# zyc-123/InstanceDiff

Measured on AMD Instinct MI355X. Metric: denoising steps/sec (256x256 bs16), higher is better.
Workload: dtype f32; 1 GPU; 256x256 1-ch synthetic, 1000-step reverse chain, batch 16 per GPU, 2 UNet fwd + reverse update per step; global_batch=16, parallelism=replicas x1 (no collective)

## Files before the change

instancediff_amd/csrc/conv1x1_x3.hip:

```cpp
#include "conv_args.h"
#include "wino_common.h"

using idiff_detail::ConvArgs;

namespace {

typedef unsigned uintx4 __attribute__((ext_vector_type(4)));
typedef __bf16 bf16x8 __attribute__((ext_vector_type(8)));

constexpr int BM = 64, CKB = 32, NT = 256;
constexpr int B_ISTR = 1088;
constexpr int B_KGSTR = 4 * B_ISTR;
constexpr int B_PLSTR = 4 * B_KGSTR;
constexpr int B_BYTES = 3 * B_PLSTR;
constexpr int A_PLSTR = 4 * 64 * 16;
constexpr int A_BYTES = 3 * A_PLSTR;
constexpr int OLD = 256 + 4;
static_assert(32 * OLD * 4 <= B_BYTES, "epilogue tile must fit in the B planes");

__host__ __device__ constexpr unsigned hi16(unsigned u) { return u & 0xffff0000u; }

__device__ __forceinline__ unsigned pack_hi(unsigned odd, unsigned even) { return __builtin_amdgcn_perm(odd, even, 0x07060302u); }

__device__ __forceinline__ void split3(const float (&x)[8], uintx4& p1, uintx4& p2, uintx4& p3) {
    unsigned u1[8], u2[8], u3[8];
#pragma unroll
    for (int c = 0; c < 8; ++c) {
        u1[c] = __builtin_bit_cast(unsigned, x[c]);
        const float r1 = x[c] - __builtin_bit_cast(float, hi16(u1[c]));
        u2[c] = __builtin_bit_cast(unsigned, r1);
        const float r2 = r1 - __builtin_bit_cast(float, hi16(u2[c]));
        u3[c] = __builtin_bit_cast(unsigned, r2);
    }
    p1 = uintx4{pack_hi(u1[1], u1[0]), pack_hi(u1[3], u1[2]), pack_hi(u1[5], u1[4]), pack_hi(u1[7], u1[6])};
    p2 = uintx4{pack_hi(u2[1], u2[0]), pack_hi(u2[3], u2[2]), pack_hi(u2[5], u2[4]), pack_hi(u2[7], u2[6])};
    p3 = uintx4{pack_hi(u3[1], u3[0]), pack_hi(u3[3], u3[2]), pack_hi(u3[5], u3[4]), pack_hi(u3[7], u3[6])};
}

using idiff_wino::scalar_ptr;

__device__ __forceinline__ floatx4 mma(const uintx4& a, const uintx4& b, const floatx4& c) {
    return __builtin_amdgcn_mfma_f32_16x16x32_bf16(__builtin_bit_cast(bf16x8, a), __builtin_bit_cast(bf16x8, b), c, 0, 0, 0);
}

template <bool UNSH>
__global__ __launch_bounds__(NT) __attribute__((amdgpu_waves_per_eu(2, 2))) void conv1x1_x3_kernel(const ConvArgs a, const unsigned short* __restrict__ wx3) {
    extern __shared__ __attribute__((aligned(16))) unsigned char smem_raw[];
    unsigned char* const Bs = smem_raw;
    unsigned char* const As = smem_raw + B_BYTES;
    float* const econst = reinterpret_cast<float*>(smem_raw + B_BYTES + A_BYTES);

    const int tid = threadIdx.x;
    const int lane = tid & 63;
    const int wave = __builtin_amdgcn_readfirstlane(tid >> 6);
    const int n16 = lane & 15, kgl = lane >> 4;

    const unsigned logical = xcd_remap(blockIdx.x, a.total_wg);
    const int cob = logical % a.ncob;
    const int tile = (logical / a.ncob) % a.ntiles;
    const int b = logical / (a.ncob * a.ntiles);
    const int co0 = cob * BM;
    const long long HW = (long long)a.Hout * a.Wout;
    const long long pix0 = (long long)tile * 256;

    {
        const int which = tid >> 6, co = co0 + (tid & 63);
        float v = 0.f;
        if (which == 0 && a.bias) v = a.bias[co];
        if (which == 1 && a.vec) v = a.vec[(long long)b * a.Cout + co];
        if (which == 2 && a.aux) v = a.aux_a[(long long)b * a.Cout + co];
        if (which == 3 && a.aux) v = a.aux_b[(long long)b * a.Cout + co];
        econst[tid] = v;
    }

    const int q = lane, kg = wave;
    const int nchunks = (a.Cin + CKB - 1) / CKB;
    floatx4 xrA[8], xrB[8];
    uintx4 ar[3];
    constexpr int RSRC_FLAGS = 0x00020000;
    const float* const s0 = a.src0 + (long long)b * a.bs0 + (UNSH ? 0 : pix0);
    const float* const s1 = a.src1 ? a.src1 + (long long)b * a.bs1 + pix0 : s0;
    const long long HWin = (long long)a.Hin * a.Win;
    const int chstride_b = (int)((UNSH ? HWin : HW) * 4);
    int xoff = q * 16;
    if (UNSH) {
        const int p = (int)pix0 + 4 * q;
        const int oy = p / a.Wout, ox = p - oy * a.Wout;
        xoff = (2 * oy * a.Win + 2 * ox) * 4;
    }
    auto load_x = [&](floatx4 (&xr)[8], int cc) {
        const int ch0 = cc * CKB + kg * 8;
        const bool valid = ch0 < a.Cin;
        if (UNSH) {
            const float* const p = s0 + (long long)(valid ? (ch0 >> 2) : 0) * HWin;
            const __amdgpu_buffer_rsrc_t rs = __builtin_amdgcn_make_buffer_rsrc(scalar_ptr(p), 0, __builtin_amdgcn_readfirstlane(valid ? 0x7fffffff : 0), RSRC_FLAGS);
#pragma unroll
            for (int c = 0; c < 8; ++c)
                xr[c] = __builtin_bit_cast(floatx4, __builtin_amdgcn_raw_buffer_load_b128(rs, xoff, (c >> 2) * chstride_b + ((c >> 1) & 1) * a.Win * 4 + (c & 1) * 16, 0));
        } else {
            const bool second = ch0 >= a.C0v;
            const float* const p = (second ? s1 : s0) + (long long)(valid ? (second ? ch0 - a.C0v : ch0) : 0) * HW;
            const __amdgpu_buffer_rsrc_t rs = __builtin_amdgcn_make_buffer_rsrc(scalar_ptr(p), 0, __builtin_amdgcn_readfirstlane(valid ? 0x7fffffff : 0), RSRC_FLAGS);
#pragma unroll
            for (int c = 0; c < 8; ++c) xr[c] = __builtin_bit_cast(floatx4, __builtin_amdgcn_raw_buffer_load_b128(rs, xoff, c * chstride_b, 0));
        }
    };
    auto load_w = [&](int cc) {
        const bool valid = cc < nchunks;
        const unsigned short* const wsrc = wx3 + ((long long)(valid ? cc : 0) * a.ncob + cob) * (A_BYTES / 2);
        const __amdgpu_buffer_rsrc_t rs = __builtin_amdgcn_make_buffer_rsrc(scalar_ptr(wsrc), 0, __builtin_amdgcn_readfirstlane(valid ? A_BYTES : 0), RSRC_FLAGS);
#pragma unroll
        for (int i = 0; i < 3; ++i) ar[i] = __builtin_bit_cast(uintx4, __builtin_amdgcn_raw_buffer_load_b128(rs, tid * 16, i * NT * 16, 0));
    };
    unsigned char* const bw = Bs + kg * B_KGSTR + q * 16;
    auto stage = [&](const floatx4 (&xr)[8]) {
#pragma unroll
        for (int i = 0; i < 4; ++i) {
            float v[8];
#pragma unroll
            for (int c = 0; c < 8; ++c) {
                if (UNSH) {
                    const int px = 2 * i + (c & 1);
                    v[c] = xr[(c >> 1) * 2 + (px >> 2)][px & 3];
                } else {
                    v[c] = xr[c][i];
                }
            }
            uintx4 p1, p2, p3;
            split3(v, p1, p2, p3);
            *reinterpret_cast<uintx4*>(bw + i * B_ISTR) = p1;
            *reinterpret_cast<uintx4*>(bw + i * B_ISTR + B_PLSTR) = p2;
            *reinterpret_cast<uintx4*>(bw + i * B_ISTR + 2 * B_PLSTR) = p3;
        }
#pragma unroll
        for (int i = 0; i < 3; ++i) reinterpret_cast<uintx4*>(As)[tid + i * NT] = ar[i];
    };

    floatx4 acc[4][4];
#pragma unroll
    for (int mi = 0; mi < 4; ++mi)
#pragma unroll
        for (int j = 0; j < 4; ++j) acc[mi][j] = floatx4{0.f, 0.f, 0.f, 0.f};
    const unsigned char* const ard = As + kgl * 1024 + n16 * 16;
    const unsigned char* const brd = Bs + kgl * B_KGSTR + (n16 & 3) * B_ISTR + (16 * wave + (n16 >> 2)) * 16;

    auto chunk = [&](int cc, auto par_tag) {
        constexpr int PAR = decltype(par_tag)::value;
        floatx4(&xr)[8] = PAR ? xrB : xrA;
        __syncthreads();
        __builtin_amdgcn_sched_barrier(0);
        stage(xr);
        __syncthreads();
        load_w(cc + 1);
        load_x(xr, cc + 2);
        __builtin_amdgcn_sched_barrier(0);
#pragma unroll
        for (int mh = 0; mh < 2; ++mh) {
            uintx4 av[2][3];
#pragma unroll
            for (int m2 = 0; m2 < 2; ++m2)
#pragma unroll
                for (int p = 0; p < 3; ++p) av[m2][p] = *reinterpret_cast<const uintx4*>(ard + p * A_PLSTR + (2 * mh + m2) * 256);
            uintx4 bv[2][3];
#pragma unroll
            for (int p = 0; p < 3; ++p) bv[0][p] = *reinterpret_cast<const uintx4*>(brd + p * B_PLSTR);
#pragma unroll
            for (int j = 0; j < 4; ++j) {
                if (j + 1 < 4) {
#pragma unroll
                    for (int p = 0; p < 3; ++p) bv[(j + 1) & 1][p] = *reinterpret_cast<const uintx4*>(brd + p * B_PLSTR + (j + 1) * 64);
                }
                const uintx4(&bj)[3] = bv[j & 1];
#pragma unroll
                for (int m2 = 0; m2 < 2; ++m2) {
                    floatx4 c = acc[2 * mh + m2][j];
                    c = mma(av[m2][2], bj[0], c);
                    c = mma(av[m2][1], bj[1], c);
                    c = mma(av[m2][0], bj[2], c);
                    c = mma(av[m2][1], bj[0], c);
                    c = mma(av[m2][0], bj[1], c);
                    c = mma(av[m2][0], bj[0], c);
                    acc[2 * mh + m2][j] = c;
                }
            }
        }
    };
    load_x(xrA, 0);
    load_w(0);
    load_x(xrB, 1);
    int cc = 0;
    for (; cc + 1 < nchunks; cc += 2) {
        chunk(cc, std::integral_constant<int, 0>{});
        chunk(cc + 1, std::integral_constant<int, 1>{});
    }
    if (cc < nchunks) chunk(cc, std::integral_constant<int, 0>{});

    float* const ot = reinterpret_cast<float*>(Bs);
    float* const outb = a.out + (long long)b * a.obs;
    const float* const resb = a.res ? a.res + (long long)b * a.rbs : nullptr;
    const float* const auxb = a.aux ? a.aux + (long long)b * a.abs_ : nullptr;
    auto rows = [&](int mb, auto res_tag, auto aux_tag) {
        constexpr bool RES = decltype(res_tag)::value, AUX = decltype(aux_tag)::value;
        constexpr int STEPS = 32 * 64 / NT;
        floatx4 nres = {0.f, 0.f, 0.f, 0.f}, naux = {0.f, 0.f, 0.f, 0.f};
        auto fetch = [&](int i) {
            const int f = tid + i * NT;
            const int row = mb * 32 + (f >> 6), c4 = (f & 63) * 4;
            const long long o = (long long)(co0 + row) * HW + pix0 + c4;
            if (RES) nres = *reinterpret_cast<const floatx4*>(resb + o);
            if (AUX) naux = *reinterpret_cast<const floatx4*>(auxb + o);
        };
        fetch(0);
        __syncthreads();
#pragma unroll
        for (int mh = 0; mh < 2; ++mh)
#pragma unroll
            for (int j = 0; j < 4; ++j)
#pragma unroll
                for (int r = 0; r < 4; ++r)
                    ot[(mh * 16 + 4 * kgl + r) * OLD + 64 * wave + 16 * j + n16] = mb ? acc[2 + mh][j][r] : acc[mh][j][r];
        __syncthreads();
#pragma unroll
        for (int i = 0; i < STEPS; ++i) {
            const int f = tid + i * NT;
            const int lrow = f >> 6, row = mb * 32 + lrow, c4 = (f & 63) * 4;
            const floatx4 cres = nres, caux = naux;
            if (i + 1 < STEPS) fetch(i + 1);
            floatx4 v = *reinterpret_cast<const floatx4*>(ot + lrow * OLD + c4);
            const float add = econst[row] + econst[BM + row];
            v = floatx4{v.x + add, v.y + add, v.z + add, v.w + add};
            if (RES) v = floatx4{v.x + cres.x, v.y + cres.y, v.z + cres.z, v.w + cres.w};
            if (AUX) {
                const float aa = econst[2 * BM + row], ab = econst[3 * BM + row];
                v = floatx4{v.x + silu_fast(aa * caux.x + ab), v.y + silu_fast(aa * caux.y + ab), v.z + silu_fast(aa * caux.z + ab),
                            v.w + silu_fast(aa * caux.w + ab)};
            }
            *reinterpret_cast<floatx4*>(outb + (long long)(co0 + row) * HW + pix0 + c4) = v;
        }
    };
    auto halves = [&](auto res_tag, auto aux_tag) {
        rows(0, res_tag, aux_tag);
        rows(1, res_tag, aux_tag);
    };
    if (resb) {
        if (auxb) halves(std::true_type{}, std::true_type{});
        else halves(std::true_type{}, std::false_type{});
    } else {
        if (auxb) halves(std::false_type{}, std::true_type{});
        else halves(std::false_type{}, std::false_type{});
    }
}

__global__ void pack_x3_kernel(const float* __restrict__ w, uintx4* __restrict__ out, int Cout, int Cin, int ncob, long long npieces) {
    for (long long i = blockIdx.x * (long long)blockDim.x + threadIdx.x; i < npieces; i += (long long)gridDim.x * blockDim.x) {
        const int co_l = i & 63;
        const int kg = (i >> 6) & 3;
        const int plane = (int)((i >> 8) % 3);
        const long long blk = i / 768;
        const int cob = (int)(blk % ncob), cc = (int)(blk / ncob);
        const int co = cob * 64 + co_l;
        float x[8];
#pragma unroll
        for (int e = 0; e < 8; ++e) {
            const int ci = cc * CKB + kg * 8 + e;
            x[e] = (co < Cout && ci < Cin) ? w[(long long)co * Cin + ci] : 0.f;
        }
        uintx4 p1, p2, p3;
        split3(x, p1, p2, p3);
        out[i] = plane == 0 ? p1 : plane == 1 ? p2 : p3;
    }
}

}

namespace idiff_detail {

bool conv1x1_x3_eligible(const ConvArgs& a, int mode) {
    const long long hw = (long long)a.Hout * a.Wout;
    if (hw % 256 || hw > (1 << 25) || a.Cout % BM || a.Cin % 8 || a.Cin < CKB || a.pro_a || a.stats) return false;
    if (mode == IDIFF_CONV_UNSHUFFLE2)
        return !a.src1 && a.Wout % 4 == 0 && a.Win == 2 * a.Wout && (long long)a.Hin * a.Win <= (1 << 25) && a.bs0 % 4 == 0 &&
               (reinterpret_cast<uintptr_t>(a.src0) & 15) == 0;
    return mode == IDIFF_CONV_NORMAL && a.Hout == 1 && a.C0v % 8 == 0;
}

int launch_conv1x1_x3(const ConvArgs& a, int mode, const void* wx3, hipStream_t st) {
    const size_t lds = B_BYTES + A_BYTES + 4 * BM * sizeof(float);
    static idiff_dyn_lds_cache lds_cache[2];
    if (const int rc = idiff_dyn_lds(lds_cache[0], conv1x1_x3_kernel<false>, lds, "conv2d(1x1 x3)")) return rc;
    if (const int rc = idiff_dyn_lds(lds_cache[1], conv1x1_x3_kernel<true>, lds, "conv2d(1x1 x3)")) return rc;
    if (mode == IDIFF_CONV_UNSHUFFLE2) hipLaunchKernelGGL(conv1x1_x3_kernel<true>, dim3(a.total_wg), dim3(NT), lds, st, a, static_cast<const unsigned short*>(wx3));
    else hipLaunchKernelGGL(conv1x1_x3_kernel<false>, dim3(a.total_wg), dim3(NT), lds, st, a, static_cast<const unsigned short*>(wx3));
    IDIFF_CHECK_LAUNCH("conv2d_fwd(1x1 x3)");
    return IDIFF_OK;
}

}

extern "C" long long idiff_conv1x1_x3_image_bytes(int Cout, int Cin) {
    return (long long)((Cin + CKB - 1) / CKB) * ((Cout + BM - 1) / BM) * A_BYTES;
}

extern "C" int idiff_pack_conv1x1_x3(const float* w, void* image, int Cout, int Cin, idiff_stream_t stream) {
    IDIFF_CHECK_ARG(w && image && Cout > 0 && Cin > 0, "pack_conv1x1_x3: bad args");
    IDIFF_CHECK_ARG((reinterpret_cast<uintptr_t>(image) & 15) == 0, "pack_conv1x1_x3: image must be 16-byte aligned");
    const int ncob = (Cout + BM - 1) / BM;
    const long long npieces = idiff_conv1x1_x3_image_bytes(Cout, Cin) / 16;
    const int grid = (int)((npieces + 255) / 256 > 4096 ? 4096 : (npieces + 255) / 256);
    hipLaunchKernelGGL(pack_x3_kernel, dim3(grid), dim3(256), 0, (hipStream_t)stream, w, static_cast<uintx4*>(image), Cout, Cin, ncob, npieces);
    IDIFF_CHECK_LAUNCH("pack_conv1x1_x3");
    return IDIFF_OK;
}
```

Baseline: 43.39 steps/s.

## Prefetch epilogue residual/aux rows through the idle x-load slots of final chunks

The x-prefetch slots that would otherwise load past the last input chunk now fetch the epilogue's residual or aux rows, so those global reads overlap the tail of the main loop instead of running serially in the epilogue. Paths that cannot reuse the slots (UNSH, or residual together with aux) fall back to loading all eight rows per half up front instead of one at a time. This hides epilogue read latency at the cost of more registers held live and more complex address logic in the x loader.

```diff
diff --git a/instancediff_amd/csrc/conv1x1_x3.hip b/instancediff_amd/csrc/conv1x1_x3.hip
--- a/instancediff_amd/csrc/conv1x1_x3.hip
+++ b/instancediff_amd/csrc/conv1x1_x3.hip
@@ -88,7 +88,13 @@
         const int oy = p / a.Wout, ox = p - oy * a.Wout;
         xoff = (2 * oy * a.Win + 2 * ox) * 4;
     }
-    auto load_x = [&](floatx4 (&xr)[8], int cc) {
+    float* const outb = a.out + (long long)b * a.obs;
+    const float* const resb = a.res ? a.res + (long long)b * a.rbs : nullptr;
+    const float* const auxb = a.aux ? a.aux + (long long)b * a.abs_ : nullptr;
+    const float* const pre = auxb ? auxb : resb;
+    const float* const pre0 = scalar_ptr((pre ? pre : s0) + (long long)(co0 + wave) * HW + pix0);
+    const int erow_stride_b = (int)(4 * HW * 4);
+    auto load_x = [&](floatx4 (&xr)[8], int cc, int mb) {
         const int ch0 = cc * CKB + kg * 8;
         const bool valid = ch0 < a.Cin;
         if (UNSH) {
@@ -98,11 +104,19 @@
             for (int c = 0; c < 8; ++c)
                 xr[c] = __builtin_bit_cast(floatx4, __builtin_amdgcn_raw_buffer_load_b128(rs, xoff, (c >> 2) * chstride_b + ((c >> 1) & 1) * a.Win * 4 + (c & 1) * 16, 0));
         } else {
+            const bool erow = cc >= nchunks;
+            const int records = __builtin_amdgcn_readfirstlane((erow ? pre != nullptr : valid) ? 0x7fffffff : 0);
             const bool second = ch0 >= a.C0v;
-            const float* const p = (second ? s1 : s0) + (long long)(valid ? (second ? ch0 - a.C0v : ch0) : 0) * HW;
-            const __amdgpu_buffer_rsrc_t rs = __builtin_amdgcn_make_buffer_rsrc(scalar_ptr(p), 0, __builtin_amdgcn_readfirstlane(valid ? 0x7fffffff : 0), RSRC_FLAGS);
-#pragma unroll
-            for (int c = 0; c < 8; ++c) xr[c] = __builtin_bit_cast(floatx4, __builtin_amdgcn_raw_buffer_load_b128(rs, xoff, c * chstride_b, 0));
+            const float* const xlo = (second ? s1 : s0) + (long long)(valid ? (second ? ch0 - a.C0v : ch0) : 0) * HW;
+            const unsigned long long lo_i = erow ? reinterpret_cast<unsigned long long>(pre0) + (unsigned long long)(mb * 32 * 4) * (unsigned long long)HW
+                                                 : reinterpret_cast<unsigned long long>(xlo);
+            const float* const lo = reinterpret_cast<const float*>(lo_i);
+            const float* const hi = lo + (long long)(erow ? 16 : 4) * HW;
+            const __amdgpu_buffer_rsrc_t rs_lo = __builtin_amdgcn_make_buffer_rsrc(scalar_ptr(lo), 0, records, RSRC_FLAGS);
+            const __amdgpu_buffer_rsrc_t rs_hi = __builtin_amdgcn_make_buffer_rsrc(scalar_ptr(hi), 0, records, RSRC_FLAGS);
+            const int stride_b = erow ? erow_stride_b : chstride_b;
+#pragma unroll
+            for (int c = 0; c < 8; ++c) xr[c] = __builtin_bit_cast(floatx4, __builtin_amdgcn_raw_buffer_load_b128(c < 4 ? rs_lo : rs_hi, xoff, (c & 3) * stride_b, 0));
         }
     };
     auto load_w = [&](int cc) {
@@ -152,7 +166,7 @@
         stage(xr);
         __syncthreads();
         load_w(cc + 1);
-        load_x(xr, cc + 2);
+        load_x(xr, cc + 2, PAR);
         __builtin_amdgcn_sched_barrier(0);
 #pragma unroll
         for (int mh = 0; mh < 2; ++mh) {
@@ -185,9 +199,9 @@
             }
         }
     };
-    load_x(xrA, 0);
+    load_x(xrA, 0, 0);
     load_w(0);
-    load_x(xrB, 1);
+    load_x(xrB, 1, 1);
     int cc = 0;
     for (; cc + 1 < nchunks; cc += 2) {
         chunk(cc, std::integral_constant<int, 0>{});
@@ -196,21 +210,21 @@
     if (cc < nchunks) chunk(cc, std::integral_constant<int, 0>{});
 
     float* const ot = reinterpret_cast<float*>(Bs);
-    float* const outb = a.out + (long long)b * a.obs;
-    const float* const resb = a.res ? a.res + (long long)b * a.rbs : nullptr;
-    const float* const auxb = a.aux ? a.aux + (long long)b * a.abs_ : nullptr;
-    auto rows = [&](int mb, auto res_tag, auto aux_tag) {
+    auto rows = [&](auto mb_tag, auto res_tag, auto aux_tag) {
+        constexpr int mb = decltype(mb_tag)::value;
         constexpr bool RES = decltype(res_tag)::value, AUX = decltype(aux_tag)::value;
+        constexpr bool LATE_RES = RES && (UNSH || AUX), LATE_AUX = AUX && UNSH;
         constexpr int STEPS = 32 * 64 / NT;
-        floatx4 nres = {0.f, 0.f, 0.f, 0.f}, naux = {0.f, 0.f, 0.f, 0.f};
-        auto fetch = [&](int i) {
+        static_assert(STEPS == 8, "a chunk slot carries the eight rows of a half");
+        const floatx4(&pr)[8] = mb ? xrB : xrA;
+        floatx4 rr[STEPS], ra[STEPS];
+#pragma unroll
+        for (int i = 0; i < STEPS; ++i) {
             const int f = tid + i * NT;
-            const int row = mb * 32 + (f >> 6), c4 = (f & 63) * 4;
-            const long long o = (long long)(co0 + row) * HW + pix0 + c4;
-            if (RES) nres = *reinterpret_cast<const floatx4*>(resb + o);
-            if (AUX) naux = *reinterpret_cast<const floatx4*>(auxb + o);
-        };
-        fetch(0);
+            const long long o = (long long)(co0 + mb * 32 + (f >> 6)) * HW + pix0 + (f & 63) * 4;
+            if (LATE_RES) rr[i] = *reinterpret_cast<const floatx4*>(resb + o);
+            if (LATE_AUX) ra[i] = *reinterpret_cast<const floatx4*>(auxb + o);
+        }
         __syncthreads();
 #pragma unroll
         for (int mh = 0; mh < 2; ++mh)
@@ -224,8 +238,7 @@
         for (int i = 0; i < STEPS; ++i) {
             const int f = tid + i * NT;
             const int lrow = f >> 6, row = mb * 32 + lrow, c4 = (f & 63) * 4;
-            const floatx4 cres = nres, caux = naux;
-            if (i + 1 < STEPS) fetch(i + 1);
+            const floatx4 cres = LATE_RES ? rr[i] : pr[i], caux = LATE_AUX ? ra[i] : pr[i];
             floatx4 v = *reinterpret_cast<const floatx4*>(ot + lrow * OLD + c4);
             const float add = econst[row] + econst[BM + row];
             v = floatx4{v.x + add, v.y + add, v.z + add, v.w + add};
@@ -239,8 +252,8 @@
         }
     };
     auto halves = [&](auto res_tag, auto aux_tag) {
-        rows(0, res_tag, aux_tag);
-        rows(1, res_tag, aux_tag);
+        rows(std::integral_constant<int, 0>{}, res_tag, aux_tag);
+        rows(std::integral_constant<int, 1>{}, res_tag, aux_tag);
     };
     if (resb) {
         if (auxb) halves(std::true_type{}, std::true_type{});
```

Measured after the change: 43.50 steps/s, median of 5. No clear change (+0.2%).
